# vkit-x/vkit

Hardware: AMD Instinct MI355X
Metric: Mpixels/s (2048^2 RGB, geo+photo chain) (higher is better)
Workload: dtype u8; 1 GPU; C3 fused chain: camera_cubic_curve remap (level 5) + gaussian_blur(sigma=1.0) + color_shift(37) + gaussion_noise(std=10.0, the numpy stream default_rng(5000 + i) drawn on the device inside every step), states built from the configs inside every step, 2048x2048x3 uint8, batch 256 per GPU; batch_per_gpu=256, image=2048x2048x3, noise_mode=tiles, states=built on the device from the configs inside every step (vkx_camera_states_dev), lanes=1

## Files before the change

### vkit_amd/csrc/fused.hip

```cpp
#include "vkx_internal.h"
#include "vkx_cell.h"
#include "vkx_color.h"

#include <float.h>
#include <memory>
#include <stdlib.h>
#include <string.h>

namespace {

constexpr int W = 64;
constexpr int RMAX = 3;
constexpr int NLDSCELL = 64;
#ifndef VKX_FUSED_NWAVES
#define VKX_FUSED_NWAVES 8
#endif
constexpr int NWAVES = VKX_FUSED_NWAVES;
constexpr int NTHREADS = 64 * NWAVES;
constexpr int ROWS_PER_WAVE = 8;
constexpr int WH = NWAVES * ROWS_PER_WAVE;
__host__ __device__ constexpr int tile_side(int R) { return (W - 2 * R) & ~3; }
__host__ __device__ constexpr int tile_height(int R) { return WH == W ? tile_side(R) : WH - 2 * R; }
#ifndef VKX_FUSED_CGROUP
#define VKX_FUSED_CGROUP 2
#endif
constexpr int CGROUP = VKX_FUSED_CGROUP;
#ifndef VKX_FUSED_WAVES_PER_EU
#define VKX_FUSED_WAVES_PER_EU 8
#endif

#define VKX_GLOBAL __attribute__((address_space(1)))
typedef const uint8_t VKX_GLOBAL *gsrc_t;
typedef uint8_t VKX_GLOBAL *gdst_t;
typedef unsigned long long u64_u1 __attribute__((aligned(1)));
typedef uint32_t u32_u1 __attribute__((aligned(1)));
typedef uint16_t u16_u1 __attribute__((aligned(1)));

struct ItemDev {
    const uint8_t *src;
    uint8_t *dst;
    const int16_t *noise;
    const int32_t *sv, *dv;
    ptrdiff_t sstride, dstride, nstride;
    int sh, sw, dh, dw;
    int rows, cols;
    int tiles_x, tiles_y;
    int cell_base;
    int R;
    int hue_on, hue_delta;
    unsigned short kq[8];
    int streak_on, streak_step, streak_thickness, streak_dash, streak_dash_step, streak_dash_gap;
    int streak_vert, streak_hori, streak_copy;
    int streak_color[3];
    float streak_alpha;
    int n_elems, pad_;
    const uint2 *noise_table;
    int noise_tiled, noise_tiles, noise_slot;
    float noise_tiles_per_sample;
    const uint2 *noise_rows;
    struct Elem {
        const void *src;
        void *dst;
        ptrdiff_t sstride, dstride;
        int cn, is_f32;
    } el[4];
};

struct ElemPack {
    ItemDev::Elem el[4];
    int n;
};

struct TileBin {
    int rmin, cmin;
    int rmax1, cmax1;
};

struct CellR {
    int ex[4], edx[4];
    short vx[4], vy[4];
    int flags, pad;
};
static_assert(sizeof(CellR) == 56, "CellR mirrors the tail of CellC");

__device__ __forceinline__ int find_item(const int *__restrict__ prefix, int n, int v)
{
    int lo = 0, hi = n - 1;
    while (lo < hi) {
        const int mid = (lo + hi + 1) >> 1;
        if (prefix[mid] <= v) lo = mid; else hi = mid - 1;
    }
    return lo;
}

constexpr int kLocalBins = 1024;

__global__ void __launch_bounds__(256) k_chain_setup(const ItemDev *__restrict__ items, const int *__restrict__ cell_prefix,
                                                     int n_items, int total_cells, int slots,
                                                     vkc::CellC *__restrict__ cells, TileBin *__restrict__ bins,
                                                     int *__restrict__ deferred )
{
    __shared__ int lbins[kLocalBins * 4];
    __shared__ int s_item, s_tiles_x, s_ty_min, s_ty_max;
    const int gid = blockIdx.x * 256 + threadIdx.x;
    const bool active = gid < total_cells;
    int ii = -1, r = 0, c = 0, tx0 = 0, tx1 = -1, ty0 = 0, ty1 = -1, tiles_x = 1;
    if (active) {
        ii = find_item(cell_prefix, n_items, gid);
        const ItemDev &it = items[ii];
        const int cell = gid - it.cell_base;
        vkc::CellC rec;
        int xmin, xmax, ymin, ymax;
        if (vkc::build_cell<vkc::kCellDirectOnly>(it.sv, it.dv, it.rows, it.cols, cell, rec, xmin, xmax, ymin, ymax)) cells[gid] = rec;
        else deferred[1 + atomicAdd(&deferred[0], 1)] = gid;
        r = cell / (it.cols - 1); c = cell - r * (it.cols - 1);
        const int Tw = tile_side(it.R), Th = tile_height(it.R);
        tx0 = (xmin - it.R) / Tw; tx1 = (xmax + it.R) / Tw; ty0 = (ymin - it.R) / Th; ty1 = (ymax + it.R) / Th;
        if (xmin - it.R < 0) tx0 = 0;
        if (ymin - it.R < 0) ty0 = 0;
        tiles_x = it.tiles_x;
        tx1 = min(tx1, tiles_x - 1);
        ty1 = min(ty1, it.tiles_y - 1);
    }
    if (threadIdx.x == 0) { s_item = ii; s_tiles_x = tiles_x; s_ty_min = INT_MAX; s_ty_max = -1; }
    __syncthreads();
    const bool local = active && ii == s_item && ty0 <= ty1 && tx0 <= tx1;
    if (local) { atomicMin(&s_ty_min, ty0); atomicMax(&s_ty_max, ty1); }
    __syncthreads();
    const int tymin = s_ty_min, nb = s_ty_max >= tymin ? (s_ty_max - tymin + 1) * s_tiles_x : 0;
    const bool use_lds = nb > 0 && nb <= kLocalBins;
    if (use_lds)
        for (int i = threadIdx.x; i < nb; i += 256) {
            lbins[4 * i] = 0x7f7f7f7f; lbins[4 * i + 1] = 0x7f7f7f7f; lbins[4 * i + 2] = 0; lbins[4 * i + 3] = 0;
        }
    __syncthreads();
    for (int ty = ty0; ty <= ty1; ty++)
        for (int tx = tx0; tx <= tx1; tx++) {
            if (local && use_lds) {
                int *b = lbins + 4 * ((ty - tymin) * tiles_x + tx);
                atomicMin(b, r); atomicMin(b + 1, c); atomicMax(b + 2, r + 1); atomicMax(b + 3, c + 1);
            } else {
                TileBin *b = bins + (size_t)ii * slots + ty * tiles_x + tx;
                atomicMin(&b->rmin, r);
                atomicMin(&b->cmin, c);
                atomicMax(&b->rmax1, r + 1);
                atomicMax(&b->cmax1, c + 1);
            }
        }
    __syncthreads();
    if (use_lds)
        for (int i = threadIdx.x; i < nb; i += 256) {
            if (lbins[4 * i + 2] == 0) continue;
            TileBin *b = bins + (size_t)s_item * slots + tymin * s_tiles_x + i;
            atomicMin(&b->rmin, lbins[4 * i]);
            atomicMin(&b->cmin, lbins[4 * i + 1]);
            atomicMax(&b->rmax1, lbins[4 * i + 2]);
            atomicMax(&b->cmax1, lbins[4 * i + 3]);
        }
}

__global__ void __launch_bounds__(64) k_chain_setup_svd(const ItemDev *__restrict__ items, const int *__restrict__ cell_prefix,
                                                        int n_items, vkc::CellC *__restrict__ cells,
                                                        const int *__restrict__ deferred)
{
    const int n = deferred[0];
    const int sub = threadIdx.x & 7;
    for (int j = blockIdx.x * 8 + (threadIdx.x >> 3); j < n; j += gridDim.x * 8) {
        const int gid = deferred[1 + j];
        const ItemDev &it = items[find_item(cell_prefix, n_items, gid)];
        vkc::CellC rec;
        int xmin, xmax, ymin, ymax;
        vkc::build_cell<vkc::kCellJacobiGroup8>(it.sv, it.dv, it.rows, it.cols, gid - it.cell_base, rec, xmin, xmax, ymin, ymax);
        if (sub == 0) cells[gid] = rec;
    }
}

__device__ __forceinline__ int div_small(int n, int d, float rcp_d)
{
    int q = (int)(((float)n + 0.5f) * rcp_d);
    const int r = n - q * d;
    q += r >= d ? 1 : 0;
    q -= r < 0 ? 1 : 0;
    return q;
}

__device__ __forceinline__ uint32_t mad_u24(uint32_t a, uint32_t b, uint32_t c)
{
    uint32_t r;
    asm("v_mad_u32_u24 %0, %1, %2, %3" : "=v"(r) : "v"(a), "v"(b), "v"(c));
    return r;
}

__device__ __forceinline__ uint32_t mad_u24_ks(uint32_t k_uniform, uint32_t b, uint32_t c)
{
    return __umul24(k_uniform, b) + c;
}
__device__ __forceinline__ uint32_t mad_u24_cs(uint32_t a, uint32_t b, uint32_t c_uniform)
{
    return __umul24(a, b) + c_uniform;
}

typedef unsigned short ushort2_t __attribute__((ext_vector_type(2)));
__device__ __forceinline__ uint32_t dot2_u16_ks(uint32_t k_uniform, uint32_t b, uint32_t c)
{
    return __builtin_amdgcn_udot2(__builtin_bit_cast(ushort2_t, k_uniform), __builtin_bit_cast(ushort2_t, b), c, false);
}

__device__ __forceinline__ uint64_t uniform64(uint64_t v)
{
    const uint32_t lo = __builtin_amdgcn_readfirstlane((uint32_t)v), hi = __builtin_amdgcn_readfirstlane((uint32_t)(v >> 32));
    return ((uint64_t)hi << 32) | lo;
}

__device__ __forceinline__ void div_pair(double nx, double ny, double de, double &qx, double &qy)
{
    bool fdx, fdy, fnx, fny;
    const double sdx = __builtin_amdgcn_div_scale(nx, de, false, &fdx);
    const double sdy = __builtin_amdgcn_div_scale(ny, de, false, &fdy);
    if (__builtin_amdgcn_ballot_w64(__double_as_longlong(sdx) != __double_as_longlong(sdy)) != 0) {
        qx = nx / de;
        qy = ny / de;
        return;
    }
    double r = __builtin_amdgcn_rcp(sdx);
// ... 556 lines not shown
        if (tiled) __syncthreads();
    }
    const int full4 = (tw >> 2) << 2;
    const bool grouped = !STREAK && (INTERIOR || ocx < full4);
    const uint32_t g4 = (uint32_t)((ocx >> 2) * 12 + (ocx & 3) * 4);
    const uint32_t k3 = grouped ? g4 : (uint32_t)(ocx * 3);
    const bool nlane = ocol && !(grouped && (ocx & 3) == 3);
    u32x2 nrow = {0u, 0u};
    if (tiled) nrow = *(const u32x2 *)(lnrow + 2 * (wave + NWAVES * (lane & 7)));
#pragma unroll
    for (int i = 0; i < ROWS_PER_WAVE; i++) {
        nzA[i] = 0; nzB[i] = 0;
        const int cy = wave + NWAVES * i;
        if (noise && nlane && cy < th) {
            const int16_t VKX_GLOBAL *np_;
            if (tiled) {
                const int16_t VKX_GLOBAL *rowp = noise + (size_t)(uint32_t)__builtin_amdgcn_readlane((int)nrow.x, i);
                const uint32_t sd = (uint32_t)__builtin_amdgcn_readlane((int)nrow.y, i);
                uint32_t off = k3;
                if ((sd & 0xffffu) < 3u * W) {
                    asm volatile("" ::: "memory");
                    off += k3 >= (sd & 0xffffu) ? (uint32_t)((int)sd >> 16) : 0u;
                }
                np_ = rowp + off;
            } else {
                np_ = noise + (ptrdiff_t)(y0 + cy) * nstride + (ptrdiff_t)x0 * 3 + (ptrdiff_t)k3;
            }
            if (grouped) {
                const unsigned long long v = *(const u64_u1 VKX_GLOBAL *)np_;
                nzA[i] = (uint32_t)v;
                nzB[i] = (uint32_t)(v >> 32);
            } else {
                nzA[i] = *(const u32_u1 VKX_GLOBAL *)np_;
                nzB[i] = *(const u16_u1 VKX_GLOBAL *)(np_ + 2);
            }
        }
    }
    uint32_t wpair[RMAX + 1];
#pragma unroll
    for (int q = 0; q <= RMAX; q++) {
        const uint32_t e0 = 2 * q < K ? kq[2 * q < 2 * RMAX + 1 ? 2 * q : 0] : 0u, e1 = 2 * q + 1 < K ? kq[2 * q + 1 < 2 * RMAX + 1 ? 2 * q + 1 : 0] : 0u;
        const uint32_t o0 = (q > 0 && 2 * q - 1 < K) ? kq[q > 0 ? 2 * q - 1 : 0] : 0u, o1 = 2 * q < K ? kq[2 * q < 2 * RMAX + 1 ? 2 * q : 0] : 0u;
        wpair[q] = (wave & 1) ? (o0 | (o1 << 16)) : (e0 | (e1 << 16));
    }
    const bool hue_on = __builtin_amdgcn_readfirstlane(ite.hue_on) != 0;
    const int hue_delta = __builtin_amdgcn_readfirstlane(ite.hue_delta);
    const int right4 = min(lane + 1, 63) << 2;
    const uint32_t dcol4 = (uint32_t)(x0 * 3) + g4;
    const bool streak_on = STREAK && ite.streak_on != 0;
    const int sxm = streak_on ? (x0 + ocx) % ite.streak_step : 0;
    const int sxd = streak_on ? (x0 + ocx) % ite.streak_dash_step : 0;
    uint32_t epx = 0;
    if constexpr (EMPTY) {
        int er = src[0], eg = src[1], eb = src[2];
        if (hue_on) hue_shift_px(lut->sdiv, lut->hdiv, hue_delta, er, eg, eb);
        epx = (uint32_t)er | ((uint32_t)eg << 8) | ((uint32_t)eb << 16);
    }
#pragma unroll
    for (int i = 0; i < ROWS_PER_WAVE; i++) {
        const int cy = wave + NWAVES * i;
        if (cy >= th) continue;
        const int gy = y0 + cy;
        uint32_t P = epx;
        if constexpr (!EMPTY) {
            if (R > 0) {
                int r, g, b;
                if constexpr (INTERIOR && RC > 0) {
                    const uint32_t *pl = own + (cy & ~1) * P_ + lane;
                    uint32_t ar = 32768u, ag = 32768u, ab = 32768u;
#pragma unroll
                    for (int q = 0; q <= RC; q++) {
                        ar = dot2_u16_ks(wpair[q], pl[q * kPairPitch], ar);
                        ag = dot2_u16_ks(wpair[q], pl[q * kPairPitch + 64], ag);
                        ab = dot2_u16_ks(wpair[q], pl[q * kPairPitch + 128], ab);
                    }
                    r = (int)(ar >> 16); g = (int)(ag >> 16); b = (int)(ab >> 16);
                } else {
                    uint32_t a0 = 0, a1 = 0, a2 = 0;
#pragma unroll
                    for (int j = 0; j < 2 * RMAX + 1; j++) {
                        if (j < K) {
                            const int yy = INTERIOR ? cy + j : vkd::reflect101(gy + j - R, dh) - wy0;
                            const uint16_t *h16 = (const uint16_t *)(own + (yy & ~1) * P_ + lane) + (yy & 1);
                            a0 += __umul24(kq[j], (uint32_t)h16[0]);
                            a1 += __umul24(kq[j], (uint32_t)h16[128]);
                            a2 += __umul24(kq[j], (uint32_t)h16[256]);
                        }
                    }
                    r = (int)((a0 + 32768u) >> 16); g = (int)((a1 + 32768u) >> 16); b = (int)((a2 + 32768u) >> 16);
                }
                if (phase_limit == 20) {
                    const int yy = INTERIOR ? cy + R : vkd::reflect101(gy, dh) - wy0;
                    const uint16_t *h16 = (const uint16_t *)(own + (yy & ~1) * P_ + lane) + (yy & 1);
                    r = h16[0] >> 8; g = h16[128] >> 8; b = h16[256] >> 8;
                }
                if (hue_on) P = vkd::hue_shift_packed(lsdiv, lhdiv, lsel, hue_delta, r, g, b);
                else P = (uint32_t)r | ((uint32_t)g << 8) | ((uint32_t)b << 16);
            } else {
                P = own[(cy + R) * P_ + lane];
                if (hue_on) P = vkd::hue_shift_packed(lsdiv, lhdiv, lsel, hue_delta, (int)(P & 0xff), (int)((P >> 8) & 0xff),
                                                      (int)((P >> 16) & 0xff));
            }
        }
        if ((STREAK || !INTERIOR) && ((noise && !grouped) || (STREAK && streak_on))) {
            int r = (int)(P & 0xff), g = (int)((P >> 8) & 0xff), b = (int)((P >> 16) & 0xff);
            if (noise) {
                r = vkd::clamp_u8((int)(int16_t)(r + (int)(nzA[i] & 0xffff)));
                g = vkd::clamp_u8((int)(int16_t)(g + (int)(nzA[i] >> 16)));
                b = vkd::clamp_u8((int)(int16_t)(b + (int)(nzB[i] & 0xffff)));
            }
            if (STREAK && streak_on) {
                const int ym = gy % ite.streak_step, yd = gy % ite.streak_dash_step;
                bool mv = ite.streak_vert && sxm < ite.streak_thickness;
                bool mh = ite.streak_hori && ym < ite.streak_thickness;
                if (ite.streak_dash) {
                    if (yd < ite.streak_dash_gap) mv = false;
                    if (sxd < ite.streak_dash_gap) mh = false;
                }
                const float w1 = ite.streak_alpha, w0 = 1.0f - w1;
                int *ch[3] = {&r, &g, &b};
#pragma unroll
                for (int c = 0; c < 3; c++) {
                    int v = *ch[c];
                    const int col = ite.streak_color[c];
                    if (mv) { const float t0 = w0 * (float)v, t1 = w1 * (float)col; v = ite.streak_copy ? col : (int)(uint8_t)(t0 + t1); }
                    if (mh) { const float t0 = w0 * (float)v, t1 = w1 * (float)col; v = ite.streak_copy ? col : (int)(uint8_t)(t0 + t1); }
                    *ch[c] = v;
                }
            }
            P = (uint32_t)r | ((uint32_t)g << 8) | ((uint32_t)b << 16);
        }
        const uint32_t Pn = (uint32_t)__builtin_amdgcn_ds_bpermute(right4, (int)P);
        gdst_t drow = dst + (ptrdiff_t)gy * dstride + (ptrdiff_t)x0 * 3;
        if (ocol) {
            const int m = ocx & 3;
            if (INTERIOR || ocx < full4) {
                if (m < 3) {
                    uint32_t wv = (P >> (8 * m)) | (Pn << (24 - 8 * m));
                    if (!STREAK && noise) wv = add_noise_u8x4(wv, nzA[i], nzB[i]);
                    const uint32_t off = (uint32_t)gy * (uint32_t)dstride + dcol4;
                    *(u32_u1 VKX_GLOBAL *)(dst + (size_t)off) = wv;
                }
            } else {
                gdst_t d = drow + ocx * 3;
                d[0] = (uint8_t)P; d[1] = (uint8_t)(P >> 8); d[2] = (uint8_t)(P >> 16);
            }
        }
    }
}

template <bool STREAK>
__global__ void __launch_bounds__(NTHREADS, VKX_FUSED_WAVES_PER_EU) k_chain_fused(const ItemDev *__restrict__ items,
                                                          const vkc::CellC *__restrict__ cells,
                                                          const TileBin *__restrict__ bins,
                                                          const HsvLut *__restrict__ lut, int phase_limit)
{
    const int slots = gridDim.x;
    const ItemDev &it = items[blockIdx.y];
    const int ntiles = it.tiles_x * it.tiles_y;
    const int per = (ntiles + 7) >> 3;
    const int run = (int)((blockIdx.x + blockIdx.y) & 7), pos = (int)(blockIdx.x >> 3);
    const int tl = run * per + pos;
    if (pos >= per || tl >= ntiles) return;
    if (phase_limit == 10) return;
    const int tile_id = (int)blockIdx.y * slots + tl;
    const TileBin bin = bins[tile_id];
    const int ty = __builtin_amdgcn_readfirstlane(div_small(tl, it.tiles_x, __builtin_amdgcn_rcpf((float)it.tiles_x)));
    const int tx = tl - ty * it.tiles_x;
    const int Tw = tile_side(it.R), Th = tile_height(it.R);
    const int wx0 = tx * Tw - it.R, wy0 = ty * Th - it.R;
    const int nc = bin.rmax1 > 0 ? max(0, bin.rmax1 - bin.rmin) * max(0, bin.cmax1 - bin.cmin) : 0;
    const bool interior = wx0 >= 0 && wy0 >= 0 && wx0 + W <= it.dw && wy0 + WH <= it.dh && nc <= NLDSCELL && phase_limit != 3;
#ifdef VKX_FUSED_CENSUS
    (void)interior;
    chain_tile<1, STREAK, VKX_FUSED_CENSUS>(it, tx, ty, cells, bin, lut, phase_limit);
    return;
#endif
    if (nc == 0) chain_tile<2, STREAK>(it, tx, ty, cells, bin, lut, phase_limit);
    else if (interior) {
        switch (it.R) {
        case 0: chain_tile<1, STREAK, 0>(it, tx, ty, cells, bin, lut, phase_limit); break;
        case 1: chain_tile<1, STREAK, 1>(it, tx, ty, cells, bin, lut, phase_limit); break;
        case 2: chain_tile<1, STREAK, 2>(it, tx, ty, cells, bin, lut, phase_limit); break;
        default: chain_tile<1, STREAK, 3>(it, tx, ty, cells, bin, lut, phase_limit); break;
        }
    } else {
        switch (it.R) {
        case 0: chain_tile<0, STREAK, 0>(it, tx, ty, cells, bin, lut, phase_limit); break;
        case 1: chain_tile<0, STREAK, 1>(it, tx, ty, cells, bin, lut, phase_limit); break;
        case 2: chain_tile<0, STREAK, 2>(it, tx, ty, cells, bin, lut, phase_limit); break;
        default: chain_tile<0, STREAK, 3>(it, tx, ty, cells, bin, lut, phase_limit); break;
        }
    }
}

__global__ void __launch_bounds__(NTHREADS, 8) k_tile_remap(const ItemDev *__restrict__ items,
                                                           const vkc::CellC *__restrict__ cells,
                                                           const TileBin *__restrict__ bins, const ElemPack pack)
{
    const int slots = gridDim.x;
    const ItemDev &it = items[blockIdx.y];
    const int ntiles = it.tiles_x * it.tiles_y;
    const int per = (ntiles + 7) >> 3;
    const int run = (int)((blockIdx.x + blockIdx.y) & 7), pos = (int)(blockIdx.x >> 3);
    const int tl = run * per + pos;
    if (pos >= per || tl >= ntiles) return;
    const int tile_id = (int)blockIdx.y * slots + tl;
    const TileBin bin = bins[tile_id];
    const int ty = __builtin_amdgcn_readfirstlane(div_small(tl, it.tiles_x, __builtin_amdgcn_rcpf((float)it.tiles_x)));
    const int tx = tl - ty * it.tiles_x;
    chain_tile<3>(it, tx, ty, cells, bin, nullptr, 0, &pack);
}

__global__ void __launch_bounds__(256) k_chain_noise_rows(const ItemDev *__restrict__ items)
{
    typedef uint32_t u32x2 __attribute__((ext_vector_type(2)));
    const ItemDev &it = items[blockIdx.y];
    if (!it.noise_rows) return;
    const uint32_t k = blockIdx.x * 256u + threadIdx.x;
    if (k >= (uint32_t)it.dh * (uint32_t)it.tiles_x) return;
    const uint32_t y = k / (uint32_t)it.tiles_x, tx = k - y * (uint32_t)it.tiles_x;
    const u32x2 VKX_GLOBAL *tab = (const u32x2 VKX_GLOBAL *)it.noise_table;
    const uint32_t T = (uint32_t)it.noise_tiles, slot = (uint32_t)it.noise_slot;
    const uint32_t i0 = (y * (uint32_t)it.dw + tx * (uint32_t)tile_side(it.R)) * 3u;
    const uint32_t g = min((uint32_t)((float)i0 * it.noise_tiles_per_sample), T - 1);
    const uint32_t gb = g > 0 ? g - 1 : 0;
    const u32x2 e0 = tab[min(gb, T)], e1 = tab[min(gb + 1, T)], e2 = tab[min(gb + 2, T)], e3 = tab[min(gb + 3, T)];
    uint32_t t;
    u32x2 a, b;
    if (i0 >= e2.x) { t = gb + 2; a = e2; b = e3; }
    else if (i0 >= e1.x) { t = gb + 1; a = e1; b = e2; }
    else { t = gb; a = e0; b = e1; }
    while (a.x > i0 && t > 0) { t--; b = a; a = tab[t]; }
    while (b.x <= i0 && t + 1 < T) { t++; a = b; b = tab[t + 1]; }
    const uint32_t before = min(b.x - i0, 0xffffu), step = slot + b.y - a.y - (b.x - a.x);
    u32x2 rec;
    rec.x = t * slot + a.y + (i0 - a.x);
    rec.y = before | (step << 16);
    ((u32x2 VKX_GLOBAL *)it.noise_rows)[k] = rec;
}

__global__ void __launch_bounds__(256) k_chain_prologue(uint32_t *__restrict__ desc_dst, const uint32_t *__restrict__ desc_src,
                                                        unsigned n_words, TileBin *__restrict__ bins, unsigned nbins,
                                                        int *__restrict__ deferred)
{
    const unsigned i = blockIdx.x * 256 + threadIdx.x;
    if (i < n_words) desc_dst[i] = desc_src[i];
    if (i < nbins) bins[i] = TileBin{0x7f7f7f7f, 0x7f7f7f7f, 0, 0};
    if (i == 0) *deferred = 0;
}

}

struct vkx_chain_plan {
    std::vector<ItemDev> dev;
    std::vector<int> prefix;
    std::vector<long long> row_prefix;
    long long ncells = 0;
    int max_tiles = 0, slots = 0;
    bool elements = false, streak = false;
    const ItemDev *d_items = nullptr;
    const int *d_cell_prefix = nullptr;
    TileBin *bins = nullptr;
    vkc::CellC *cells = nullptr;
    int *deferred = nullptr;
    const HsvLut *lut = nullptr;
};

void vkx_chain_plan_free(vkx_chain_plan *p) { delete p; }
int vkx_chain_plan_items(const vkx_chain_plan *p) { return (int)p->dev.size(); }

int vkx_chain_plan_setup(vkx_ctx *ctx, vkx_chain_plan *p)
{
    const int n_items = (int)p->dev.size();
    int rc;
    vkx_scratch *s_cells = p->elements ? &ctx->cells : &ctx->chain_cells;
    vkx_scratch *s_bins = p->elements ? &ctx->owner : &ctx->chain_bins;
    vkx_scratch *s_misc = p->elements ? &ctx->misc : &ctx->chain_misc;
    const size_t cells_bytes = sizeof(vkc::CellC) * (size_t)p->ncells;
    if ((rc = vkx_scratch_reserve(ctx, s_cells, cells_bytes + sizeof(int) * ((size_t)p->ncells + 1)))) return rc;
    p->slots = ((p->max_tiles + 7) / 8) * 8;
    const size_t nbins = (size_t)p->slots * n_items;
    if (n_items > 65535) return VKX_ERR_UNSUPPORTED;
    if ((rc = vkx_scratch_reserve(ctx, s_bins, sizeof(TileBin) * nbins))) return rc;
    const size_t items_bytes = sizeof(ItemDev) * (size_t)n_items, prefix_bytes = sizeof(int) * p->prefix.size();
    vkx_tables tab(ctx);
    const size_t items_off = tab.add(items_bytes), prefix_off = tab.add(prefix_bytes), misc_bytes = tab.bytes;
    if ((rc = vkx_scratch_reserve(ctx, s_misc, misc_bytes))) return rc;
    if (!p->elements && (rc = vkx_hsv_tables(ctx, (const void **)&p->lut))) return rc;
    unsigned char *misc = (unsigned char *)s_misc->ptr;
    if ((rc = tab.take())) return rc;
    memcpy(tab.at<char>(items_off), p->dev.data(), items_bytes);
    memcpy(tab.at<char>(prefix_off), p->prefix.data(), prefix_bytes);
    p->d_items = (const ItemDev *)(misc + items_off);
    p->d_cell_prefix = (const int *)(misc + prefix_off);
    p->bins = (TileBin *)s_bins->ptr;
    p->cells = (vkc::CellC *)s_cells->ptr;
    p->deferred = (int *)((unsigned char *)s_cells->ptr + cells_bytes);
    {
        const unsigned char *ring_dev = tab.mapped();
        if (!ring_dev) { vkx_set_error("%s: the descriptor ring is not mapped into the device's address space", __func__); return VKX_ERR_HIP; }
        const size_t n_words = (misc_bytes + 3) / 4;
        VKX_TIMED(ctx, "k_chain_prologue");
        k_chain_prologue<<<vkx_blocks(std::max(n_words, nbins), 256), 256, 0, ctx->stream>>>((uint32_t *)misc, (const uint32_t *)ring_dev,
                                                                                            (unsigned)n_words, p->bins, (unsigned)nbins, p->deferred);
        VKX_LAUNCH_CHECK();
    }
    { VKX_TIMED(ctx, "k_chain_setup"); k_chain_setup<<<vkx_blocks((size_t)p->ncells, 256), 256, 0, ctx->stream>>>(p->d_items, p->d_cell_prefix, n_items, (int)p->ncells, p->slots, p->cells, p->bins, p->deferred); }
    VKX_LAUNCH_CHECK();
    { VKX_TIMED(ctx, "k_chain_setup_svd"); k_chain_setup_svd<<<128, 64, 0, ctx->stream>>>(p->d_items, p->d_cell_prefix, n_items, p->cells, p->deferred); }
    VKX_LAUNCH_CHECK();
    return VKX_OK;
}

int vkx_chain_plan_noise_rows(vkx_ctx *ctx, vkx_chain_plan *p, int first, int count)
{
    if (p->row_prefix.empty() || count <= 0) return VKX_OK;
    long long most = 0;
    for (int i = first; i < first + count; i++) most = std::max(most, p->row_prefix[i + 1] - p->row_prefix[i]);
    if (most <= 0) return VKX_OK;
    VKX_TIMED(ctx, "k_chain_noise_rows");
    k_chain_noise_rows<<<dim3(vkx_blocks((size_t)most, 256), count), 256, 0, ctx->stream>>>(p->d_items + first);
    VKX_LAUNCH_CHECK();
    return VKX_OK;
}

int vkx_chain_plan_tiles(vkx_ctx *ctx, vkx_chain_plan *p, int first, int count)
{
    if (count <= 0) return VKX_OK;
    static const int phase_limit = [] { const char *e = getenv("VKX_FUSED_PHASES"); return e ? atoi(e) : 0; }();
    const ItemDev *items = p->d_items + first;
    const TileBin *bins = p->bins + (size_t)first * p->slots;
    const dim3 grid(p->slots, count);
    if (p->elements) {
        VKX_TIMED(ctx, "k_tile_remap");
        ElemPack pack;
        memset(&pack, 0, sizeof(pack));
        pack.n = p->dev[first].n_elems;
        for (int e = 0; e < 4; e++) pack.el[e] = p->dev[first].el[e];
        k_tile_remap<<<grid, NTHREADS, kFusedLds, ctx->stream>>>(items, p->cells, bins, pack);
    } else {
        VKX_TIMED_MAJOR(ctx, "k_chain_fused");
        if (p->streak) k_chain_fused<true><<<grid, NTHREADS, kFusedLds, ctx->stream>>>(items, p->cells, bins, p->lut, phase_limit);
        else k_chain_fused<false><<<grid, NTHREADS, kFusedLds, ctx->stream>>>(items, p->cells, bins, p->lut, phase_limit);
    }
    VKX_LAUNCH_CHECK();
    return VKX_OK;
}

int vkx_chain_plan_build(vkx_ctx *ctx, const vkx_chain_item *items, int n_items, vkx_chain_plan **out)
{
    *out = nullptr;
    if (n_items <= 0) return VKX_OK;
    std::unique_ptr<vkx_chain_plan> plan(new vkx_chain_plan());
    std::vector<ItemDev> &dev = plan->dev;
    dev.resize(n_items);
    plan->prefix.resize((size_t)n_items + 1);
    int *cell_prefix = plan->prefix.data();
    std::vector<long long> &row_prefix = plan->row_prefix;
    row_prefix.assign((size_t)n_items + 1, 0);
    long long tiles = 0, ncells = 0;
    int max_tiles = 0;
    for (int i = 0; i < n_items; i++) {
        const vkx_chain_item &it = items[i];
        if (it.blur_ksize > 2 * RMAX + 1 || (it.blur_ksize > 1 && (it.blur_ksize & 1) == 0)) return VKX_ERR_UNSUPPORTED;
        if (it.sh > 32767 || it.sw > 32767 || it.dh > 32767 || it.dw > 32767) return VKX_ERR_UNSUPPORTED;
        if (it.rows < 2 || it.cols < 2) return VKX_ERR_UNSUPPORTED;
        if (it.blur_ksize > 1 && (it.dh == 1 || it.dw == 1)) return VKX_ERR_UNSUPPORTED;
        ItemDev &d = dev[i];
        memset(&d, 0, sizeof(d));
        d.src = it.src; d.dst = it.dst; d.noise = it.noise; d.sv = it.src_vertices; d.dv = it.dst_vertices;
        d.sstride = it.src_stride; d.dstride = it.dst_stride; d.nstride = it.noise_stride_el;
        d.noise_table = nullptr; d.noise_tiled = 0; d.noise_tiles = 0; d.noise_slot = 0; d.noise_tiles_per_sample = 0.f;
        d.noise_rows = nullptr;
        if (it.noise && it.noise_tiled) {
            const long long n = (long long)it.dh * it.dw * 3;
            if (n > 0x7fffffffLL) return VKX_ERR_UNSUPPORTED;
            const vkx_np_tiles_shape shape = vkx_np_tiles_shape_of(n);
            if (shape.n_tiles * shape.slot_elems > 0xffffffffLL) return VKX_ERR_UNSUPPORTED;
            d.noise = (const int16_t *)((const unsigned char *)it.noise + shape.slots_offset);
            d.noise_table = (const uint2 *)((const unsigned char *)it.noise + shape.table_offset);
            d.noise_tiled = 1; d.noise_tiles = (int)shape.n_tiles; d.noise_slot = shape.slot_elems;
            d.noise_tiles_per_sample = (float)(1.0 / shape.samples_per_tile);
        }
        d.sh = it.sh; d.sw = it.sw; d.dh = it.dh; d.dw = it.dw; d.rows = it.rows; d.cols = it.cols;
        d.R = it.blur_ksize > 1 ? it.blur_ksize / 2 : 0;
        const int Tw = tile_side(d.R), Th = tile_height(d.R);
        d.tiles_x = (it.dw + Tw - 1) / Tw; d.tiles_y = (it.dh + Th - 1) / Th;
        d.cell_base = (int)ncells;
        d.hue_on = it.hue_enabled; d.hue_delta = it.hue_delta;
        d.streak_on = it.streak_enabled && it.streak_alpha != 0.0 && (it.streak_enable_vert || it.streak_enable_hori);
        if (it.streak_enabled) {
            if (it.streak_thickness + it.streak_gap <= 0) return VKX_ERR_UNSUPPORTED;
            d.streak_thickness = it.streak_thickness;
            d.streak_step = it.streak_thickness + it.streak_gap;
            d.streak_dash = it.streak_dash_thickness > 0 && it.streak_dash_gap > 0;
            d.streak_dash_step = d.streak_dash ? it.streak_dash_thickness + it.streak_dash_gap : 1;
            d.streak_dash_gap = it.streak_dash_gap;
            d.streak_vert = it.streak_enable_vert; d.streak_hori = it.streak_enable_hori;
            d.streak_copy = it.streak_alpha == 1.0;
            d.streak_alpha = (float)it.streak_alpha;
            for (int c = 0; c < 3; c++) d.streak_color[c] = it.streak_color[c];
        }
        for (int k = 0; k < 8; k++) d.kq[k] = 0;
        if (d.R > 0 && vkx_gaussian_kernel_q8_host(it.blur_ksize, it.blur_sigma, d.kq)) return VKX_ERR_UNSUPPORTED;
        for (int k = 0; k < d.R; k++)
            if (d.kq[k] != d.kq[2 * d.R - k]) return VKX_ERR_UNSUPPORTED;
        if (it.src_stride <= 0 || it.src_stride >= (1 << 24) || (long long)it.sh * it.src_stride + 8 > 0xffffffffLL) return VKX_ERR_UNSUPPORTED;
        if (it.dst_stride <= 0 || (long long)it.dh * it.dst_stride > 0xffffffffLL) return VKX_ERR_UNSUPPORTED;
        cell_prefix[i] = (int)ncells;
        row_prefix[i + 1] = row_prefix[i] + (d.noise_tiled ? (long long)it.dh * d.tiles_x : 0);
        tiles += (long long)d.tiles_x * d.tiles_y;
        if (d.tiles_x * d.tiles_y > max_tiles) max_tiles = d.tiles_x * d.tiles_y;
        ncells += (long long)(it.rows - 1) * (it.cols - 1);
        if (tiles > 0x3fffffff || ncells > 0x3fffffff) return VKX_ERR_UNSUPPORTED;
        plan->streak = plan->streak || d.streak_on != 0;
    }
    cell_prefix[n_items] = (int)ncells;
    if (n_items > 65535) return VKX_ERR_UNSUPPORTED;
    if (row_prefix[n_items] > 0) {
        int rc = vkx_scratch_reserve(ctx, &ctx->noise_rows, (size_t)row_prefix[n_items] * sizeof(uint2));
        if (rc) return rc;
        for (int i = 0; i < n_items; i++)
            if (dev[i].noise_tiled) dev[i].noise_rows = (const uint2 *)ctx->noise_rows.ptr + row_prefix[i];
    } else {
        row_prefix.clear();
    }
    plan->ncells = ncells;
    plan->max_tiles = max_tiles;
    *out = plan.release();
    return VKX_OK;
}

int vkx_chain_plan_setup_aside(vkx_ctx *ctx, vkx_chain_plan *p, hipEvent_t *done)
{
    static const int aside_env = [] { const char *e = getenv("VKX_CHAIN_SETUP_ASIDE"); return e ? (e[0] == '0' ? 0 : 1) : -1; }();
    constexpr size_t kAsideMinItems = 16;
    const bool aside = aside_env >= 0 ? aside_env != 0 : p->dev.size() >= kAsideMinItems;
    *done = nullptr;
    if (!aside) {
        if (ctx->lattices_armed) {
            vkx_device_guard guard(ctx);
            VKX_HIP(hipStreamWaitEvent(ctx->stream, ctx->lattices_ready, 0));
            ctx->lattices_armed = false;
        }
        return vkx_chain_plan_setup(ctx, p);
    }
    int rc;
    hipStream_t main_stream = ctx->stream;
    hipStream_t side = vkx_stream_by_id(ctx, VKX_STREAM_COPY_OUT, &rc);
    if (rc) return rc;
    vkx_device_guard guard(ctx);
    if (ctx->lattices_armed) {
        VKX_HIP(hipStreamWaitEvent(side, ctx->lattices_ready, 0));
        ctx->lattices_armed = false;
    } else if ((rc = vkx_stream_order(ctx, side, main_stream))) return rc;
    if (ctx->chain_done) VKX_HIP(hipStreamWaitEvent(side, ctx->chain_done, 0));
    ctx->stream = side;
    rc = vkx_chain_plan_setup(ctx, p);
    ctx->stream = main_stream;
    if (rc) return rc;
    if (!ctx->chain_setup_done) VKX_HIP(hipEventCreateWithFlags(&ctx->chain_setup_done, hipEventDisableTiming));
    VKX_HIP(hipEventRecord(ctx->chain_setup_done, side));
    *done = ctx->chain_setup_done;
    return VKX_OK;
}

int vkx_chain_mark_done(vkx_ctx *ctx, hipStream_t stream)
{
    if (!ctx->chain_done) VKX_HIP(hipEventCreateWithFlags(&ctx->chain_done, hipEventDisableTiming));
    VKX_HIP(hipEventRecord(ctx->chain_done, stream));
    return VKX_OK;
}

int vkx_chain_fused_try(vkx_ctx *ctx, const vkx_chain_item *items, int n_items)
{
    vkx_chain_plan *raw = nullptr;
    int rc = vkx_chain_plan_build(ctx, items, n_items, &raw);
    if (rc || !raw) return rc;
    std::unique_ptr<vkx_chain_plan, void (*)(vkx_chain_plan *)> plan(raw, vkx_chain_plan_free);
    hipStream_t main_stream = ctx->stream;
    auto schedule = [&]() -> int {
        int rc;
        hipEvent_t setup_done = nullptr;
        if ((rc = vkx_chain_plan_setup_aside(ctx, raw, &setup_done))) return rc;
        if (setup_done) VKX_HIP(hipStreamWaitEvent(ctx->stream, setup_done, 0));
        if ((rc = vkx_chain_plan_noise_rows(ctx, raw, 0, n_items))) return rc;
        if ((rc = vkx_chain_plan_tiles(ctx, raw, 0, n_items))) return rc;
        vkx_device_guard guard(ctx);
        return vkx_chain_mark_done(ctx, ctx->stream);
    };
    rc = schedule();
    if (rc) vkx_ctx_join_streams(ctx, main_stream);
    return rc;
}

int vkx_tile_remap_try(vkx_ctx *ctx, const vkx_elem *elems, int n_elems, int sh, int sw, const int32_t *src_vertices,
                       const int32_t *dst_vertices, int rows, int cols, int dh, int dw)
{
    if (n_elems < 1 || n_elems > 4 || rows < 2 || cols < 2) return VKX_ERR_UNSUPPORTED;
    if (sh > 32767 || sw > 32767 || dh > 32767 || dw > 32767 || sh < 1 || sw < 1 || dh < 1 || dw < 1) return VKX_ERR_UNSUPPORTED;
    vkx_chain_plan plan;
    plan.dev.resize(1);
    plan.prefix.resize(2);
    std::vector<int> &prefix = plan.prefix;
    ItemDev &d = plan.dev[0];
    memset(&d, 0, sizeof(d));
    d.sv = src_vertices; d.dv = dst_vertices;
    d.sh = sh; d.sw = sw; d.dh = dh; d.dw = dw; d.rows = rows; d.cols = cols;
    d.R = 0;
    const int Tw = tile_side(0), Th = tile_height(0);
    d.tiles_x = (dw + Tw - 1) / Tw; d.tiles_y = (dh + Th - 1) / Th;
    d.cell_base = 0;
    d.n_elems = n_elems;
    for (int e = 0; e < n_elems; e++) {
        if (!elems[e].src || !elems[e].dst) return VKX_ERR_UNSUPPORTED;
        if (!elems[e].is_f32 && elems[e].cn != 1 && elems[e].cn != 3 && elems[e].cn != 4) return VKX_ERR_UNSUPPORTED;
        if (elems[e].is_f32 && elems[e].cn != 1) return VKX_ERR_UNSUPPORTED;
        d.el[e].src = elems[e].src; d.el[e].dst = elems[e].dst;
        d.el[e].sstride = elems[e].src_stride; d.el[e].dstride = elems[e].dst_stride;
        d.el[e].cn = elems[e].cn; d.el[e].is_f32 = elems[e].is_f32;
    }
    const long long ncells = (long long)(rows - 1) * (cols - 1);
    if ((long long)d.tiles_x * d.tiles_y > 0x3fffffff || ncells > 0x3fffffff) return VKX_ERR_UNSUPPORTED;
    prefix[0] = 0; prefix[1] = (int)ncells;
    plan.elements = true;
    plan.ncells = ncells;
    plan.max_tiles = d.tiles_x * d.tiles_y;
    int rc = vkx_chain_plan_setup(ctx, &plan);
    if (rc) return rc;
    return vkx_chain_plan_tiles(ctx, &plan, 0, 1);
}
```

Measured before the change: 71670 Mpixels/s.

## Split fused chain launch into interior, rim and overflow kernels

The single fused chain kernel is replaced, for large batches, by three launches. One covers the interior rectangle of tiles using only the fast LDS path and appends tiles with too many cells to an overflow list. One handles the border rim tiles on the generic path, and a persistent kernel processes the overflow list. This removes per-tile interior/border divergence and keeps the interior kernel specialized, at the cost of extra launches, an atomic-built work list and extra scratch memory.

```diff
diff --git a/vkit_amd/csrc/fused.hip b/vkit_amd/csrc/fused.hip
--- a/vkit_amd/csrc/fused.hip
+++ b/vkit_amd/csrc/fused.hip
@@ -45,6 +45,7 @@
     int sh, sw, dh, dw;
     int rows, cols;
     int tiles_x, tiles_y;
+    int rect_x0, rect_y0, rect_w, rect_h;
     int cell_base;
     int R;
     int hue_on, hue_delta;
@@ -70,6 +71,21 @@
     ItemDev::Elem el[4];
     int n;
 };
+
+struct TileRect {
+    int x0, y0, x1, y1;
+    __host__ __device__ bool empty() const { return x1 < x0 || y1 < y0; }
+};
+__host__ __device__ inline TileRect interior_rect(int dw, int dh, int R)
+{
+    const int Tw = tile_side(R), Th = tile_height(R);
+    TileRect r;
+    r.x0 = (R + Tw - 1) / Tw;
+    r.y0 = (R + Th - 1) / Th;
+    r.x1 = dw - W + R >= 0 ? (dw - W + R) / Tw : -1;
+    r.y1 = dh - WH + R >= 0 ? (dh - WH + R) / Th : -1;
+    return r;
+}
 
 struct TileBin {
     int rmin, cmin;
@@ -932,6 +948,106 @@
 template <bool STREAK>
 __global__ void __launch_bounds__(NTHREADS, VKX_FUSED_WAVES_PER_EU) k_chain_fused(const ItemDev *__restrict__ items,
                                                           const vkc::CellC *__restrict__ cells,
+                                                          const TileBin *__restrict__ bins, int bin_slots,
+                                                          int *__restrict__ over_count, int2 *__restrict__ over_list, int over_slots,
+                                                          const HsvLut *__restrict__ lut, int phase_limit)
+{
+    const ItemDev &it = items[blockIdx.y];
+    const int rw = it.rect_w;
+    const int nrect = rw * it.rect_h;
+    const int per = (nrect + 7) >> 3;
+    const int run = (int)((blockIdx.x + blockIdx.y) & 7), pos = (int)(blockIdx.x >> 3);
+    const int rl = run * per + pos;
+    if (pos >= per || rl >= nrect) return;
+    if (phase_limit == 10) return;
+    const int ry = __builtin_amdgcn_readfirstlane(div_small(rl, rw, __builtin_amdgcn_rcpf((float)rw)));
+    const int tx = it.rect_x0 + rl - ry * rw, ty = it.rect_y0 + ry;
+    const int tl = ty * it.tiles_x + tx;
+    const TileBin bin = bins[(size_t)blockIdx.y * bin_slots + tl];
+    const int nc = bin.rmax1 > 0 ? max(0, bin.rmax1 - bin.rmin) * max(0, bin.cmax1 - bin.cmin) : 0;
+#ifdef VKX_FUSED_CENSUS
+    (void)nc;
+    chain_tile<1, STREAK, VKX_FUSED_CENSUS>(it, tx, ty, cells, bin, lut, phase_limit);
+    return;
+#endif
+    if (nc == 0) chain_tile<2, STREAK>(it, tx, ty, cells, bin, lut, phase_limit);
+    else if (nc <= NLDSCELL && phase_limit != 3) {
+        switch (it.R) {
+        case 0: chain_tile<1, STREAK, 0>(it, tx, ty, cells, bin, lut, phase_limit); break;
+        case 1: chain_tile<1, STREAK, 1>(it, tx, ty, cells, bin, lut, phase_limit); break;
+        case 2: chain_tile<1, STREAK, 2>(it, tx, ty, cells, bin, lut, phase_limit); break;
+        default: chain_tile<1, STREAK, 3>(it, tx, ty, cells, bin, lut, phase_limit); break;
+        }
+    } else if (threadIdx.x == 0) {
+        const int k = atomicAdd(over_count, 1);
+        if (k < over_slots) over_list[k] = make_int2((int)blockIdx.y, tl);
+    }
+}
+
+template <bool STREAK>
+__global__ void __launch_bounds__(NTHREADS, VKX_FUSED_WAVES_PER_EU) k_chain_fused_rim(const ItemDev *__restrict__ items,
+                                                          const vkc::CellC *__restrict__ cells,
+                                                          const TileBin *__restrict__ bins, int bin_slots,
+                                                          const HsvLut *__restrict__ lut, int phase_limit)
+{
+    if (phase_limit == 10) return;
+    const ItemDev &it = items[blockIdx.y];
+    const int tiles_x = it.tiles_x, rw = it.rect_w, rh = it.rect_h;
+    const int nrim = tiles_x * it.tiles_y - rw * rh;
+    const int per = (nrim + 7) >> 3;
+    const int run = (int)((blockIdx.x + blockIdx.y) & 7), pos = (int)(blockIdx.x >> 3);
+    const int q = run * per + pos;
+    if (pos >= per || q >= nrim) return;
+    int tl;
+    const int top = it.rect_y0 * tiles_x, bottom = (it.tiles_y - it.rect_y0 - rh) * tiles_x;
+    if (rw * rh == 0 || q < top) tl = q;
+    else if (q < top + bottom) tl = q - top + (it.rect_y0 + rh) * tiles_x;
+    else {
+        const int m = q - top - bottom, side = tiles_x - rw;
+        const int r = __builtin_amdgcn_readfirstlane(div_small(m, side, __builtin_amdgcn_rcpf((float)side)));
+        const int c = m - r * side;
+        tl = (it.rect_y0 + r) * tiles_x + (c < it.rect_x0 ? c : c + rw);
+    }
+    const TileBin bin = bins[(size_t)blockIdx.y * bin_slots + tl];
+    const int ty = __builtin_amdgcn_readfirstlane(div_small(tl, tiles_x, __builtin_amdgcn_rcpf((float)tiles_x)));
+    const int tx = tl - ty * tiles_x;
+    const int nc = bin.rmax1 > 0 ? max(0, bin.rmax1 - bin.rmin) * max(0, bin.cmax1 - bin.cmin) : 0;
+    if (nc == 0) chain_tile<2, STREAK>(it, tx, ty, cells, bin, lut, phase_limit);
+    else {
+        switch (it.R) {
+        case 0: chain_tile<0, STREAK, 0>(it, tx, ty, cells, bin, lut, phase_limit); break;
+        case 1: chain_tile<0, STREAK, 1>(it, tx, ty, cells, bin, lut, phase_limit); break;
+        case 2: chain_tile<0, STREAK, 2>(it, tx, ty, cells, bin, lut, phase_limit); break;
+        default: chain_tile<0, STREAK, 3>(it, tx, ty, cells, bin, lut, phase_limit); break;
+        }
+    }
+}
+
+constexpr int kOverGrid = 512;
+template <bool STREAK>
+__global__ void __launch_bounds__(NTHREADS, 4) k_chain_fused_over(const ItemDev *__restrict__ items,
+                                                          const vkc::CellC *__restrict__ cells,
+                                                          const TileBin *__restrict__ bins, int bin_slots,
+                                                          const int *__restrict__ over_count, const int2 *__restrict__ over_list,
+                                                          int over_slots, const HsvLut *__restrict__ lut, int phase_limit)
+{
+    const int n_over = min(*over_count, over_slots);
+    if ((int)blockIdx.x >= n_over || phase_limit == 10) return;
+    for (int k = (int)blockIdx.x; k < n_over; k += (int)gridDim.x) {
+        const int2 e = over_list[k];
+        const int img = __builtin_amdgcn_readfirstlane(e.x), tl = __builtin_amdgcn_readfirstlane(e.y);
+        const ItemDev &it = items[img];
+        const TileBin bin = bins[(size_t)img * bin_slots + tl];
+        const int tiles_x = __builtin_amdgcn_readfirstlane(it.tiles_x);
+        const int ty = __builtin_amdgcn_readfirstlane(div_small(tl, tiles_x, __builtin_amdgcn_rcpf((float)tiles_x)));
+        chain_tile<0, STREAK>(it, tl - ty * tiles_x, ty, cells, bin, lut, phase_limit);
+        __syncthreads();
+    }
+}
+
+template <bool STREAK>
+__global__ void __launch_bounds__(NTHREADS, VKX_FUSED_WAVES_PER_EU) k_chain_fused_whole(const ItemDev *__restrict__ items,
+                                                          const vkc::CellC *__restrict__ cells,
                                                           const TileBin *__restrict__ bins,
                                                           const HsvLut *__restrict__ lut, int phase_limit)
 {
@@ -951,11 +1067,6 @@
     const int wx0 = tx * Tw - it.R, wy0 = ty * Th - it.R;
     const int nc = bin.rmax1 > 0 ? max(0, bin.rmax1 - bin.rmin) * max(0, bin.cmax1 - bin.cmin) : 0;
     const bool interior = wx0 >= 0 && wy0 >= 0 && wx0 + W <= it.dw && wy0 + WH <= it.dh && nc <= NLDSCELL && phase_limit != 3;
-#ifdef VKX_FUSED_CENSUS
-    (void)interior;
-    chain_tile<1, STREAK, VKX_FUSED_CENSUS>(it, tx, ty, cells, bin, lut, phase_limit);
-    return;
-#endif
     if (nc == 0) chain_tile<2, STREAK>(it, tx, ty, cells, bin, lut, phase_limit);
     else if (interior) {
         switch (it.R) {
@@ -1022,11 +1133,12 @@
 
 __global__ void __launch_bounds__(256) k_chain_prologue(uint32_t *__restrict__ desc_dst, const uint32_t *__restrict__ desc_src,
                                                         unsigned n_words, TileBin *__restrict__ bins, unsigned nbins,
-                                                        int *__restrict__ deferred)
+                                                        int *__restrict__ deferred, int *__restrict__ over_count, unsigned n_over)
 {
     const unsigned i = blockIdx.x * 256 + threadIdx.x;
     if (i < n_words) desc_dst[i] = desc_src[i];
     if (i < nbins) bins[i] = TileBin{0x7f7f7f7f, 0x7f7f7f7f, 0, 0};
+    if (i < n_over) over_count[i] = 0;
     if (i == 0) *deferred = 0;
 }
 
@@ -1038,12 +1150,15 @@
     std::vector<long long> row_prefix;
     long long ncells = 0;
     int max_tiles = 0, slots = 0;
+    int rect_slots = 0;
     bool elements = false, streak = false;
     const ItemDev *d_items = nullptr;
     const int *d_cell_prefix = nullptr;
     TileBin *bins = nullptr;
     vkc::CellC *cells = nullptr;
     int *deferred = nullptr;
+    int *over_count = nullptr;
+    int2 *over_list = nullptr;
     const HsvLut *lut = nullptr;
 };
 
@@ -1062,7 +1177,8 @@
     p->slots = ((p->max_tiles + 7) / 8) * 8;
     const size_t nbins = (size_t)p->slots * n_items;
     if (n_items > 65535) return VKX_ERR_UNSUPPORTED;
-    if ((rc = vkx_scratch_reserve(ctx, s_bins, sizeof(TileBin) * nbins))) return rc;
+    const size_t over_ints = p->elements ? 0 : (size_t)n_items * (2 + 2 * (size_t)p->rect_slots);
+    if ((rc = vkx_scratch_reserve(ctx, s_bins, sizeof(TileBin) * nbins + sizeof(int) * over_ints))) return rc;
     const size_t items_bytes = sizeof(ItemDev) * (size_t)n_items, prefix_bytes = sizeof(int) * p->prefix.size();
     vkx_tables tab(ctx);
     const size_t items_off = tab.add(items_bytes), prefix_off = tab.add(prefix_bytes), misc_bytes = tab.bytes;
@@ -1075,6 +1191,8 @@
     p->d_items = (const ItemDev *)(misc + items_off);
     p->d_cell_prefix = (const int *)(misc + prefix_off);
     p->bins = (TileBin *)s_bins->ptr;
+    p->over_count = (int *)(p->bins + nbins);
+    p->over_list = (int2 *)(p->over_count + n_items + (n_items & 1));
     p->cells = (vkc::CellC *)s_cells->ptr;
     p->deferred = (int *)((unsigned char *)s_cells->ptr + cells_bytes);
     {
@@ -1083,7 +1201,8 @@
         const size_t n_words = (misc_bytes + 3) / 4;
         VKX_TIMED(ctx, "k_chain_prologue");
         k_chain_prologue<<<vkx_blocks(std::max(n_words, nbins), 256), 256, 0, ctx->stream>>>((uint32_t *)misc, (const uint32_t *)ring_dev,
-                                                                                            (unsigned)n_words, p->bins, (unsigned)nbins, p->deferred);
+                                                                                            (unsigned)n_words, p->bins, (unsigned)nbins, p->deferred,
+                                                                                            p->over_count, p->elements ? 0u : (unsigned)n_items);
         VKX_LAUNCH_CHECK();
     }
     { VKX_TIMED(ctx, "k_chain_setup"); k_chain_setup<<<vkx_blocks((size_t)p->ncells, 256), 256, 0, ctx->stream>>>(p->d_items, p->d_cell_prefix, n_items, (int)p->ncells, p->slots, p->cells, p->bins, p->deferred); }
@@ -1111,8 +1230,8 @@
     static const int phase_limit = [] { const char *e = getenv("VKX_FUSED_PHASES"); return e ? atoi(e) : 0; }();
     const ItemDev *items = p->d_items + first;
     const TileBin *bins = p->bins + (size_t)first * p->slots;
-    const dim3 grid(p->slots, count);
     if (p->elements) {
+        const dim3 grid(p->slots, count);
         VKX_TIMED(ctx, "k_tile_remap");
         ElemPack pack;
         memset(&pack, 0, sizeof(pack));
@@ -1120,9 +1239,46 @@
         for (int e = 0; e < 4; e++) pack.el[e] = p->dev[first].el[e];
         k_tile_remap<<<grid, NTHREADS, kFusedLds, ctx->stream>>>(items, p->cells, bins, pack);
     } else {
+        int most_rect = 0, most_rim = 0;
+        long long all_rect = 0, all_tiles = 0;
+        for (int i = first; i < first + count; i++) {
+            const ItemDev &d = p->dev[i];
+            most_rect = std::max(most_rect, d.rect_w * d.rect_h);
+            all_rect += d.rect_w * d.rect_h;
+            all_tiles += (long long)d.tiles_x * d.tiles_y;
+            most_rim = std::max(most_rim, d.tiles_x * d.tiles_y - d.rect_w * d.rect_h);
+        }
+        int *over_count = p->over_count + first;
+        int2 *over_list = p->over_list + (size_t)first * p->rect_slots;
+        const int over_slots = (int)std::min<long long>((long long)count * p->rect_slots, INT_MAX);
         VKX_TIMED_MAJOR(ctx, "k_chain_fused");
-        if (p->streak) k_chain_fused<true><<<grid, NTHREADS, kFusedLds, ctx->stream>>>(items, p->cells, bins, p->lut, phase_limit);
-        else k_chain_fused<false><<<grid, NTHREADS, kFusedLds, ctx->stream>>>(items, p->cells, bins, p->lut, phase_limit);
+        constexpr long long kSplitMinTiles = 65536;
+        const char *split_e = getenv("VKX_CHAIN_SPLIT");
+        const int split_env = split_e && split_e[0] ? (split_e[0] == '0' ? 0 : 1) : -1;
+        if (split_env >= 0 ? split_env == 0 : all_tiles < kSplitMinTiles) {
+            const dim3 grid(p->slots, count);
+            if (p->streak) k_chain_fused_whole<true><<<grid, NTHREADS, kFusedLds, ctx->stream>>>(items, p->cells, bins, p->lut, phase_limit);
+            else k_chain_fused_whole<false><<<grid, NTHREADS, kFusedLds, ctx->stream>>>(items, p->cells, bins, p->lut, phase_limit);
+            VKX_LAUNCH_CHECK();
+            return VKX_OK;
+        }
+        if (most_rect > 0) {
+            const dim3 grid_rect((most_rect + 7) / 8 * 8, count);
+            if (p->streak) k_chain_fused<true><<<grid_rect, NTHREADS, kFusedLds, ctx->stream>>>(items, p->cells, bins, p->slots, over_count, over_list, over_slots, p->lut, phase_limit);
+            else k_chain_fused<false><<<grid_rect, NTHREADS, kFusedLds, ctx->stream>>>(items, p->cells, bins, p->slots, over_count, over_list, over_slots, p->lut, phase_limit);
+            VKX_LAUNCH_CHECK();
+        }
+        if (most_rim > 0) {
+            const dim3 grid_rim((most_rim + 7) / 8 * 8, count);
+            if (p->streak) k_chain_fused_rim<true><<<grid_rim, NTHREADS, kFusedLds, ctx->stream>>>(items, p->cells, bins, p->slots, p->lut, phase_limit);
+            else k_chain_fused_rim<false><<<grid_rim, NTHREADS, kFusedLds, ctx->stream>>>(items, p->cells, bins, p->slots, p->lut, phase_limit);
+            VKX_LAUNCH_CHECK();
+        }
+        if (most_rect > 0) {
+            const dim3 grid_over((unsigned)std::min<long long>((all_rect + 1) / 2, kOverGrid));
+            if (p->streak) k_chain_fused_over<true><<<grid_over, NTHREADS, kFusedLds, ctx->stream>>>(items, p->cells, bins, p->slots, over_count, over_list, over_slots, p->lut, phase_limit);
+            else k_chain_fused_over<false><<<grid_over, NTHREADS, kFusedLds, ctx->stream>>>(items, p->cells, bins, p->slots, over_count, over_list, over_slots, p->lut, phase_limit);
+        }
     }
     VKX_LAUNCH_CHECK();
     return VKX_OK;
@@ -1140,7 +1296,7 @@
     std::vector<long long> &row_prefix = plan->row_prefix;
     row_prefix.assign((size_t)n_items + 1, 0);
     long long tiles = 0, ncells = 0;
-    int max_tiles = 0;
+    int max_tiles = 0, max_rect = 0;
     for (int i = 0; i < n_items; i++) {
         const vkx_chain_item &it = items[i];
         if (it.blur_ksize > 2 * RMAX + 1 || (it.blur_ksize > 1 && (it.blur_ksize & 1) == 0)) return VKX_ERR_UNSUPPORTED;
@@ -1167,6 +1323,9 @@
         d.R = it.blur_ksize > 1 ? it.blur_ksize / 2 : 0;
         const int Tw = tile_side(d.R), Th = tile_height(d.R);
         d.tiles_x = (it.dw + Tw - 1) / Tw; d.tiles_y = (it.dh + Th - 1) / Th;
+        const TileRect rect = interior_rect(it.dw, it.dh, d.R);
+        if (!rect.empty()) { d.rect_x0 = rect.x0; d.rect_y0 = rect.y0; d.rect_w = rect.x1 - rect.x0 + 1; d.rect_h = rect.y1 - rect.y0 + 1; }
+        max_rect = std::max(max_rect, d.rect_w * d.rect_h);
         d.cell_base = (int)ncells;
         d.hue_on = it.hue_enabled; d.hue_delta = it.hue_delta;
         d.streak_on = it.streak_enabled && it.streak_alpha != 0.0 && (it.streak_enable_vert || it.streak_enable_hori);
@@ -1208,6 +1367,7 @@
     }
     plan->ncells = ncells;
     plan->max_tiles = max_tiles;
+    plan->rect_slots = (max_rect + 7) / 8 * 8;
     *out = plan.release();
     return VKX_OK;
 }
```

Measured after the change: 72780 Mpixels/s (median of 6 runs). 1.02x the previous value.
